# cbacary/MoDeGPT

Measured on AMD Instinct MI355X. Metric: transformer layers compressed/sec (covariance+decomp+rebuild), Llama-3-8B @30%, higher is better.
Workload: dtype f64 from int8 MFMA digit planes, exact route: nine plane pairs + fp64 remainder sums, nothing truncated (error <= 5e-15 per call: fp64 rounding)

## Files before the change

### modegpt_amd/csrc/cov_i8_exact.hip

```cpp
#include <algorithm>

#include "cov_i8.hpp"

namespace mdg {

struct __attribute__((aligned(16))) LoEntry {
  double v;
  unsigned off, aux;
};

namespace {

constexpr int LO_CHUNK_STEPS = 64;
constexpr int LO_CAP = 128;
constexpr double LO_ROUND = 8421504.0 / 16777216.0;
constexpr int EXACT_OVERFLOW = offsetof(SharedBlock, exact_overflow) / sizeof(int), EXACT_RAN = offsetof(SharedBlock, exact_ran) / sizeof(int),
              EXACT_MODE = offsetof(SharedBlock, exact_mode) / sizeof(int);
#ifndef MDG_LO_SPARSE_MEAN
#define MDG_LO_SPARSE_MEAN 32
#endif
#ifndef MDG_LO_SPARSE_MAX
#define MDG_LO_SPARSE_MAX 256
#endif
constexpr int LO_SPARSE_MAX = MDG_LO_SPARSE_MAX;
constexpr int LO_SUB = 4, LO_RCAP = 8 * LO_SPARSE_MAX;
constexpr int LO_TILE = 128, LO_PITCH = LO_TILE + 1;

struct LoProblem {
  const bf16_t* x;
  int64_t ld;
  const signed char* planes;
  const unsigned char* zmask;
  const int* emax;
  LoEntry* entries;
  int* counts;
  double* sigma;
  int64_t ld_sigma;
  bf16_t* xd;
  int n, block;
  LoEntry* rentries;
  int* rtotals;
  int tile0[3];
  int pairs;
};
struct LoArgs {
  LoProblem prob[MAX_PROBLEMS];
  int nprob, nk, nch, tiles[3];
  int64_t n_tokens;
  int always;
  const int* route_flag;
  int* state;
};
__device__ __forceinline__ int* lo_totals(const LoProblem& pr, int nch) { return pr.counts + (int64_t)pr.n * nch; }
constexpr int LO_AUTO_MIN_N = 4096;
__device__ __forceinline__ bool lo_offered(const LoArgs& a) {
  if (a.always) return true;
  if (a.prob[0].n >= LO_AUTO_MIN_N && !a.prob[0].block) return true;
  for (int p = 0; p < a.nprob; p++)
    if ((a.route_flag[p] & 3) == 1) return true;
  return false;
}

__global__ __launch_bounds__(64) void i8_extract_lo_kernel(LoArgs a) {
  const LoProblem& pr = a.prob[blockIdx.z];
  const int64_t groups = pr.n / 32;
  const int G = blockIdx.x, ch = blockIdx.y, lane = threadIdx.x;
  if (!lo_offered(a)) return;
  if (blockIdx.x == 0 && blockIdx.y == 0 && blockIdx.z == 0 && lane == 0) a.state[EXACT_RAN] = 1;
  if (G >= groups || (a.route_flag[blockIdx.z] & 2)) return;
  const int col = G * 32 + (lane & 31);
  LoEntry* out = pr.entries + ((int64_t)col * a.nch + ch) * LO_CAP;
  const double scale = ldexp(1.0, (pr.emax[col] & 255) - 172);
  int count = 0;
  const int kt1 = min(a.nk, (ch + 1) * LO_CHUNK_STEPS);
  for (int kt = ch * LO_CHUNK_STEPS; kt < kt1; kt++) {
    const unsigned m = pr.zmask[(int64_t)kt * groups + G];
    if ((m >> 3) == 0) continue;
    const i32x4 zero = (i32x4)0;
    const i32x4 d3 = *((const i32x4*)(pr.planes + ((3 * groups + G) * (int64_t)a.nk + kt) * 1024) + lane);
    const i32x4 d4 = (m >> 4) ? *((const i32x4*)(pr.planes + ((4 * groups + G) * (int64_t)a.nk + kt) * 1024) + lane) : zero;
    const i32x4 d5 = (m >> 5) ? *((const i32x4*)(pr.planes + ((5 * groups + G) * (int64_t)a.nk + kt) * 1024) + lane) : zero;
    const unsigned tok0 = (unsigned)kt * KS + (lane >> 5) * 16;
    int L[16], mine = 0;
#pragma unroll
    for (int q = 0; q < 16; q++) {
      const int sh = 8 * (q & 3);
      L[q] = (int)(signed char)((unsigned)d3[q >> 2] >> sh) * 65536 + (int)(signed char)((unsigned)d4[q >> 2] >> sh) * 256 +
             (int)(signed char)((unsigned)d5[q >> 2] >> sh);
      mine += L[q] != 0;
    }
    if (__ballot(mine != 0) == 0) continue;
    const int other = __shfl_xor(mine, 32);
    int at = count + ((lane >> 5) ? other : 0);
#pragma unroll
    for (int q = 0; q < 16; q++)
      if (L[q] != 0) {
        if (at < LO_CAP) out[at] = LoEntry{(double)L[q] * scale, (tok0 + q) * (unsigned)(pr.ld * 2), (tok0 + q) * (unsigned)(pr.n * 2)};
        at++;
      }
    count += mine + other;
  }
  if (lane < 32) {
    pr.counts[(int64_t)col * a.nch + ch] = min(count, LO_CAP);
    if (count > LO_CAP) a.state[EXACT_OVERFLOW] = 1;
  }
}

__global__ __launch_bounds__(64) void i8_compact_lo_kernel(LoArgs a) {
  if (!lo_offered(a) || a.state[EXACT_OVERFLOW] != 0) return;
  const LoProblem& pr = a.prob[blockIdx.y];
  const int col = blockIdx.x, lane = threadIdx.x;
  if (col >= pr.n || (a.route_flag[blockIdx.y] & 2)) return;
  const int* counts = pr.counts + (int64_t)col * a.nch;
  LoEntry* base = pr.entries + (int64_t)col * a.nch * LO_CAP;
  int total = 0;
  for (int ch = 0; ch < a.nch; ch++) {
    const int cnt = counts[ch];
    const LoEntry* src = base + (int64_t)ch * LO_CAP;
    if (total != ch * LO_CAP)
      for (int i = 0; i < cnt; i += 64) {
        LoEntry e = LoEntry{0., 0u, 0u};
        if (i + lane < cnt) e = src[i + lane];
        if (i + lane < cnt) base[total + i + lane] = e;
      }
    total += cnt;
  }
  if (lane == 0) lo_totals(pr, a.nch)[col] = total;
}

typedef unsigned u32x4 __attribute__((ext_vector_type(4)));
constexpr int LO_SPARSE_MEAN = MDG_LO_SPARSE_MEAN;
__global__ __launch_bounds__(1024) void i8_lo_mode_kernel(LoArgs a) {
  if (!lo_offered(a) || a.state[EXACT_OVERFLOW] != 0) return;
  __shared__ long long sums[16];
  __shared__ int maxs[16];
  long long sum = 0, cols = 0;
  int mx = 0;
  for (int p = 0; p < a.nprob; p++) {
    if (a.route_flag[p] & 2) continue;
    const LoProblem& pr = a.prob[p];
    cols += pr.n;
    for (int c = threadIdx.x; c < pr.n; c += 1024) {
      const int t = lo_totals(pr, a.nch)[c];
      sum += t;
      mx = max(mx, t);
    }
  }
  for (int o = 32; o; o >>= 1) {
    sum += __shfl_xor(sum, o);
    mx = max(mx, __shfl_xor(mx, o));
  }
  if ((threadIdx.x & 63) == 0) { sums[threadIdx.x >> 6] = sum; maxs[threadIdx.x >> 6] = mx; }
  __syncthreads();
  if (threadIdx.x == 0) {
    for (int w = 1; w < 16; w++) { sum += sums[w]; mx = max(mx, maxs[w]); }
    a.state[EXACT_MODE] = (mx <= LO_SPARSE_MAX && sum <= LO_SPARSE_MEAN * cols) ? 1 : 2;
  }
}

__global__ __launch_bounds__(64) void i8_residue_lo_kernel(LoArgs a) {
  if (a.state[EXACT_MODE] != 1) return;
  const LoProblem& pr = a.prob[blockIdx.y];
  const int id = blockIdx.x, lane = threadIdx.x;
  if (id >= pr.n / 32 * LO_SUB || (a.route_flag[blockIdx.y] & 2)) return;
  const int G = id / LO_SUB, sub = id % LO_SUB;
  LoEntry* out = pr.rentries + (int64_t)id * LO_RCAP;
  int at = 0;
  for (int k = 0; k < 8; k++) {
    const int col = G * 32 + 4 * k + sub;
    const int cnt = lo_totals(pr, a.nch)[col];
    for (int i = lane; i < cnt; i += 64) {
      LoEntry e = pr.entries[(int64_t)col * a.nch * LO_CAP + i];
      e.aux = 4 * k + sub;
      out[at + i] = e;
    }
    at += cnt;
  }
  if (lane == 0) pr.rtotals[id] = at;
}

template <class EL, bool RELU>
__global__ __launch_bounds__(256) void i8_copy_xd_kernel(LoArgs a) {
  if (a.state[EXACT_MODE] != 2) return;
  const LoProblem& pr = a.prob[blockIdx.y];
  if (a.route_flag[blockIdx.y] & 2) return;
  const int64_t per_row = pr.n / 8, total = a.n_tokens * per_row;
  for (int64_t i = (int64_t)blockIdx.x * 256 + threadIdx.x; i < total; i += (int64_t)gridDim.x * 256) {
    const int64_t t = i / per_row, c = (i - t * per_row) * 8;
    typedef unsigned u32x4u __attribute__((ext_vector_type(4), aligned(2)));
    const u32x4u v = *(const u32x4u*)(pr.x + t * pr.ld + c);
    *(u32x4*)(pr.xd + t * pr.n + c) = (u32x4){relu_pair<EL, RELU>(v[0]), relu_pair<EL, RELU>(v[1]), relu_pair<EL, RELU>(v[2]), relu_pair<EL, RELU>(v[3])};
  }
}
template <class EL, bool RELU>
__global__ __launch_bounds__(64) void i8_patch_xd_kernel(LoArgs a) {
  if (a.state[EXACT_MODE] != 2) return;
  const LoProblem& pr = a.prob[blockIdx.y];
  const int col = blockIdx.x, lane = threadIdx.x;
  if (col >= pr.n || (a.route_flag[blockIdx.y] & 2)) return;
  const int total = lo_totals(pr, a.nch)[col];
  const LoEntry* list = pr.entries + (int64_t)col * a.nch * LO_CAP;
  for (int i = lane; i < total; i += 64) {
    const LoEntry e = list[i];
    const double xd = EL::to_f64(*(const bf16_t*)((const char*)pr.x + e.off + 2 * col)) - e.v;
    *(bf16_t*)((char*)pr.xd + e.aux + 2 * col) = (bf16_t)EL::from_f64(xd);
  }
}

__device__ __forceinline__ void lds_add_f64(double* p, double v) {
  __hip_atomic_fetch_add(p, v, __ATOMIC_RELAXED, __HIP_MEMORY_SCOPE_WORKGROUP);
}
__device__ __forceinline__ int lo_perm(int i) { return (i >> 1) + 64 * (i & 1); }

constexpr int LO_UN = 32;
struct LoFirst {
  int cnt;
  LoEntry m;
};
__device__ __forceinline__ LoFirst lo_first(const LoProblem& pr, const int G, const int sub, const int lane) {
  const int list_id = G * LO_SUB + sub;
  LoFirst f;
  f.cnt = __builtin_amdgcn_readfirstlane(pr.rtotals[list_id]);
  f.m = LoEntry{0., 0u, 0u};
  if (f.cnt > 0) {
    f.m = pr.rentries[(int64_t)list_id * LO_RCAP + min(lane & (LO_UN - 1), f.cnt - 1)];
    if ((lane & (LO_UN - 1)) >= f.cnt) f.m.v = 0.;
  }
  return f;
}
template <class EL, bool RELU, bool COLS>
__device__ __forceinline__ void lo_events(const LoProblem& pr, const int nch, const int G, const int sub, const int partner0, const int g,
                                          const int lane, double* acc, const LoFirst& first) {
  const unsigned short* xs = (const unsigned short*)pr.x;
  unsigned lim_a = 0, lim_b = 0;
  double qa = 1., qb = 1., ia = 1., ib = 1.;
  if (COLS) {
    const int ea = pr.emax[partner0 + 2 * lane] & 255, eb = pr.emax[partner0 + 2 * lane + 1] & 255;
    qa = ldexp(1.0, ea - 148);
    qb = ldexp(1.0, eb - 148);
    ia = 1.0 / qa;
    ib = 1.0 / qb;
    lim_a = EL::deep_limit(ea);
    lim_b = EL::deep_limit(eb);
  }
  const int list_id = G * LO_SUB + sub;
  const int cnt = first.cnt;
  const LoEntry* list = pr.rentries + (int64_t)list_id * LO_RCAP;
  auto fetch = [&](int k, LoEntry& m) {
    m = list[min(k * LO_UN + (lane & (LO_UN - 1)), cnt - 1)];
    if (k * LO_UN + (lane & (LO_UN - 1)) >= cnt) m.v = 0.;
  };
  auto issue = [&](const LoEntry& m, unsigned (&xv)[LO_UN]) {
#pragma unroll
    for (int u = 0; u < LO_UN; u++) {
      const unsigned off = (unsigned)__builtin_amdgcn_readlane((int)m.off, u);
      const unsigned short* row = (const unsigned short*)((const char*)xs + off) + partner0 + 2 * lane;
      xv[u] = relu_pair<EL, RELU>(pr.pairs ? *(const unsigned*)row : ((unsigned)row[0] | ((unsigned)row[1] << 16)));
    }
  };
  auto multiply = [&](const LoEntry& m, const unsigned (&xv)[LO_UN]) {
#pragma unroll
    for (int u = 0; u < LO_UN; u++) {
      const double v = __hiloint2double(__builtin_amdgcn_readlane(__double2hiint(m.v), u), __builtin_amdgcn_readlane(__double2loint(m.v), u));
      const int col = __builtin_amdgcn_readlane((int)m.aux, u);
      double pa = EL::to_f64(xv[u] & 0xFFFFu), pb = EL::to_f64(xv[u] >> 16);
      if (COLS) {
        const bool deep = ((xv[u] & 0x7FFFu) - 1u < lim_a - 1u) || (((xv[u] >> 16) & 0x7FFFu) - 1u < lim_b - 1u);
        if (__ballot(deep)) {
          pa = floor(pa * ia + LO_ROUND) * qa;
          pb = floor(pb * ib + LO_ROUND) * qb;
        }
        lds_add_f64(acc + lane * LO_PITCH + lo_perm(g * 32 + col), v * pa);
        lds_add_f64(acc + (64 + lane) * LO_PITCH + lo_perm(g * 32 + col), v * pb);
      } else {
        lds_add_f64(acc + lo_perm(g * 32 + col) * LO_PITCH + lane, v * pa);
        lds_add_f64(acc + lo_perm(g * 32 + col) * LO_PITCH + 64 + lane, v * pb);
      }
    }
  };
  if (cnt == 0) return;
  const int nb = (cnt + LO_UN - 1) / LO_UN;
  LoEntry mA = first.m, mB;
  unsigned xA[LO_UN], xB[LO_UN];
  issue(mA, xA);
  for (int k = 0; k < nb; k += 2) {
    if (k + 1 < nb) {
      fetch(k + 1, mB);
      issue(mB, xB);
    }
    __builtin_amdgcn_sched_barrier(0);
    multiply(mA, xA);
    if (k + 1 >= nb) break;
    if (k + 2 < nb) {
      fetch(k + 2, mA);
      issue(mA, xA);
    }
    __builtin_amdgcn_sched_barrier(0);
    multiply(mB, xB);
  }
}

constexpr int LO_THREADS = 1024;
template <class EL, bool RELU>
__global__ __launch_bounds__(LO_THREADS) void i8_lo_product_kernel(LoArgs a) {
  extern __shared__ __attribute__((aligned(16))) double lo_acc[];
  if (a.state[EXACT_RAN] != 1 || a.state[EXACT_OVERFLOW] != 0 || a.state[EXACT_MODE] != 1) return;
  int p = 0;
  while (p + 1 < a.nprob && (int)blockIdx.x >= a.prob[p + 1].tile0[2]) p++;
  if (a.route_flag[p] & 2) return;
  const LoProblem& pr = a.prob[p];
  const int t = blockIdx.x - pr.tile0[2];
  int bi, bj;
  if (pr.block) {
    bi = bj = t;
  } else {
    bi = (int)((sqrtf(8.f * t + 1.f) - 1.f) * 0.5f);
    while ((bi + 1) * (bi + 2) / 2 <= t) bi++;
    while (bi * (bi + 1) / 2 > t) bi--;
    bj = t - bi * (bi + 1) / 2;
  }
  const int tid = threadIdx.x, lane = tid & 63;
  const int wave = __builtin_amdgcn_readfirstlane(tid >> 6);
  const int g = wave & 3, sub = wave >> 2;
  int any = 0;
  if (tid < 8 * LO_SUB) any = pr.rtotals[(tid < 4 * LO_SUB ? 4 * bi * LO_SUB : 4 * bj * LO_SUB - 4 * LO_SUB) + tid];
  if (!__syncthreads_or(any)) return;
  const LoFirst first_rows = lo_first(pr, 4 * bi + g, sub, lane), first_cols = lo_first(pr, 4 * bj + g, sub, lane);
  for (int i = tid; i < LO_TILE * LO_PITCH; i += LO_THREADS) lo_acc[i] = 0.;
  __syncthreads();
  lo_events<EL, RELU, false>(pr, a.nch, 4 * bi + g, sub, bj * LO_TILE, g, lane, lo_acc, first_rows);
  __syncthreads();
  lo_events<EL, RELU, true>(pr, a.nch, 4 * bj + g, sub, bi * LO_TILE, g, lane, lo_acc, first_cols);
  __syncthreads();
  constexpr int PER = LO_TILE * LO_TILE / LO_THREADS;
  const int c = tid % LO_TILE, col = bj * LO_TILE + c;
  const int e_col = col < pr.n ? pr.emax[col] : EMAX_COLUMN_OUT;
  double* s[PER];
  double old[PER], v[PER];
#pragma unroll
  for (int u = 0; u < PER; u++) {
    const int r = tid / LO_TILE + u * (LO_THREADS / LO_TILE), row = bi * LO_TILE + r;
    v[u] = lo_acc[lo_perm(r) * LO_PITCH + lo_perm(c)];
    const bool ours = col <= row && row < pr.n && v[u] != 0. && !((pr.emax[row] | e_col) & EMAX_COLUMN_OUT);
    s[u] = ours ? pr.sigma + (int64_t)row * pr.ld_sigma + col - (pr.block ? row / pr.block * pr.block : 0) : nullptr;
    old[u] = ours ? *s[u] : 0.;
  }
#pragma unroll
  for (int u = 0; u < PER; u++)
    if (s[u]) *s[u] = old[u] + v[u];
}

#ifndef MDG_LW_UN
#define MDG_LW_UN 8
#endif
#ifndef MDG_LW_OCC
#define MDG_LW_OCC 0
#endif
#if MDG_LW_OCC
#define LW_OCC_ATTR __attribute__((amdgpu_waves_per_eu(MDG_LW_OCC, MDG_LW_OCC)))
#else
#define LW_OCC_ATTR
#endif
constexpr int LW_COLS = 8, LW_BLOCK = 64 * LW_COLS, LW_UN = MDG_LW_UN, LW_GROUP = 16, LW_TP = LW_GROUP + 1;
template <class EL, bool RELU, bool TR>
__global__ __launch_bounds__(LO_THREADS) LW_OCC_ATTR void i8_lo_wide_kernel(LoArgs a) {
  if (a.state[EXACT_RAN] != 1 || a.state[EXACT_OVERFLOW] != 0 || a.state[EXACT_MODE] != 2) return;
  int p = 0;
  while (p + 1 < a.nprob && (int)blockIdx.x >= a.prob[p + 1].tile0[TR]) p++;
  if (a.route_flag[p] & 2) return;
  const LoProblem& pr = a.prob[p];
  const int n = pr.n, nG = n / LW_GROUP;
  constexpr int PER = LW_BLOCK / LW_GROUP;
  int t = blockIdx.x - pr.tile0[TR], G, P = 0;
  if (pr.block) {
    G = t;
  } else {
    for (;;) {
      const int cnt = TR ? min(nG, PER * (P + 1)) : nG - PER * P;
      if (t < cnt) break;
      t -= cnt;
      P++;
    }
    G = TR ? t : PER * P + t;
  }
  const int lane = threadIdx.x & 63;
  const int wave = __builtin_amdgcn_readfirstlane(threadIdx.x >> 6);
  const char* const xs = TR ? (const char*)pr.xd : (const char*)pr.x;
  typedef unsigned u32x4u __attribute__((ext_vector_type(4), aligned(2)));
  __shared__ double tr_tile[TR ? LW_BLOCK * LW_TP : 1];
  const int r = G * LW_GROUP + wave;
  const int total = __builtin_amdgcn_readfirstlane(lo_totals(pr, a.nch)[r]);
  const bool r_ours = total != 0 && !(pr.emax[r] & EMAX_COLUMN_OUT);
  const LoEntry* list = pr.entries + (int64_t)r * a.nch * LO_CAP;
  LoEntry m0 = LoEntry{0., 0u, 0u};
  if (r_ours) {
    m0 = list[min(lane, min(total, 64) - 1)];
    if (lane >= total) m0.v = 0.;
  }
  {
    const int p0 = pr.block ? G * LW_GROUP / pr.block * pr.block : P * LW_BLOCK;
    const int pend = pr.block ? p0 + pr.block : min(n, p0 + LW_BLOCK);
    const int c0 = p0 + LW_COLS * lane;
    unsigned mine = 0;
#pragma unroll
    for (int j = 0; j < LW_COLS; j++)
      if (c0 + j < pend && !(pr.emax[c0 + j] & EMAX_COLUMN_OUT) && (TR ? c0 + j >= r : c0 + j <= r)) mine |= 1u << j;
    const unsigned lane_off = (unsigned)(c0 + LW_COLS <= pend ? c0 : p0) * 2u;
    const bool walk = r_ours && __ballot(mine != 0) != 0;
    double acc[LW_COLS];
#pragma unroll
    for (int j = 0; j < LW_COLS; j++) acc[j] = 0.;
    if (walk) {
      for (int sb = 0; sb < total; sb += 64) {
        const int len = min(64, total - sb);
        LoEntry m = m0;
        if (sb) {
          m = list[sb + min(lane, len - 1)];
          if (lane >= len) m.v = 0.;
        }
        const unsigned moff = TR ? m.aux : m.off;
        u32x4 xa[LW_UN], xb[LW_UN];
        auto issue = [&](int b, u32x4 (&xv)[LW_UN]) {
#pragma unroll
          for (int u = 0; u < LW_UN; u++) {
            const unsigned o = (unsigned)__builtin_amdgcn_readlane((int)moff, b * LW_UN + u) + lane_off;
            const u32x4u q = *(const u32x4u*)(xs + o);
            xv[u] = (u32x4){q[0], q[1], q[2], q[3]};
          }
        };
        auto multiply = [&](int b, const u32x4 (&xv)[LW_UN]) {
#pragma unroll
          for (int u = 0; u < LW_UN; u++) {
            const double v = __hiloint2double(__builtin_amdgcn_readlane(__double2hiint(m.v), b * LW_UN + u),
                                              __builtin_amdgcn_readlane(__double2loint(m.v), b * LW_UN + u));
#pragma unroll
            for (int q = 0; q < 4; q++) {
              const unsigned w = TR ? xv[u][q] : relu_pair<EL, RELU>(xv[u][q]);
              acc[2 * q] = fma(v, EL::lo_f64(w), acc[2 * q]);
              acc[2 * q + 1] = fma(v, EL::hi_f64(w), acc[2 * q + 1]);
            }
          }
        };
        const int nb = (len + LW_UN - 1) / LW_UN;
        issue(0, xa);
        for (int b = 0; b < nb; b += 2) {
          __builtin_amdgcn_sched_barrier(0);
          if (b + 1 < nb) issue(b + 1, xb);
          __builtin_amdgcn_sched_barrier(0);
          multiply(b, xa);
          if (b + 1 >= nb) break;
          __builtin_amdgcn_sched_barrier(0);
          if (b + 2 < nb) issue(b + 2, xa);
          __builtin_amdgcn_sched_barrier(0);
          multiply(b + 1, xb);
        }
      }
    }
    if (!TR) {
      if (!walk) return;
      double* s[LW_COLS];
      double old[LW_COLS];
#pragma unroll
      for (int j = 0; j < LW_COLS; j++) {
        s[j] = (mine >> j & 1) ? pr.sigma + (int64_t)r * pr.ld_sigma + c0 + j - (pr.block ? r / pr.block * pr.block : 0) : nullptr;
        old[j] = s[j] ? *s[j] : 0.;
      }
#pragma unroll
      for (int j = 0; j < LW_COLS; j++)
        if (s[j]) *s[j] = old[j] + acc[j];
      return;
    }
#pragma unroll
    for (int j = 0; j < LW_COLS; j++) tr_tile[(LW_COLS * lane + j) * LW_TP + wave] = (walk && (mine >> j & 1)) ? acc[j] : 0.;
    __syncthreads();
    {
      const int i = p0 + (threadIdx.x >> 1), half = threadIdx.x & 1;
      if (i < pend && !(pr.emax[i] & EMAX_COLUMN_OUT)) {
        double v[8], old[8];
        double* s[8];
#pragma unroll
        for (int k = 0; k < 8; k++) {
          const int col = G * LW_GROUP + 8 * half + k;
          v[k] = tr_tile[(i - p0) * LW_TP + 8 * half + k];
          s[k] = (v[k] != 0. && col <= i) ? pr.sigma + (int64_t)i * pr.ld_sigma + col - (pr.block ? i / pr.block * pr.block : 0) : nullptr;
          old[k] = s[k] ? *s[k] : 0.;
        }
#pragma unroll
        for (int k = 0; k < 8; k++)
          if (s[k]) *s[k] = old[k] + v[k];
      }
    }
  }
}

template <bool TR>
void launch_lo_wide(const I8Call& c, const LoArgs& lo) {
  const dim3 grid((unsigned)lo.tiles[TR]), block(LO_THREADS);
  if (c.f16) {
    if (c.relu) hipLaunchKernelGGL((i8_lo_wide_kernel<F16Elem, true, TR>), grid, block, 0, c.st, lo);
    else hipLaunchKernelGGL((i8_lo_wide_kernel<F16Elem, false, TR>), grid, block, 0, c.st, lo);
  } else {
    if (c.relu) hipLaunchKernelGGL((i8_lo_wide_kernel<Bf16Elem, true, TR>), grid, block, 0, c.st, lo);
    else hipLaunchKernelGGL((i8_lo_wide_kernel<Bf16Elem, false, TR>), grid, block, 0, c.st, lo);
  }
}

int lo_chunks(int64_t T) { return (int)ceil_div(ceil_div(T, (int64_t)KS), (int64_t)LO_CHUNK_STEPS); }

LoArgs lo_args(const I8Call& c, bool always) {
  LoArgs lo;
  lo.nprob = c.count;
  lo.nk = c.nk;
  lo.nch = lo_chunks(c.n_tokens);
  lo.route_flag = c.shared->route_flag;
  lo.state = c.shared->reserved;
  lo.always = always ? 1 : 0;
  lo.n_tokens = c.n_tokens;
  int tiles[3] = {0, 0, 0};
  for (int i = 0; i < c.count; i++) {
    const I8Stat& s = c.stat[i];
    LoProblem& l = lo.prob[i];
    l.x = s.x; l.ld = s.ld;
    l.planes = s.planes; l.zmask = s.zmask; l.emax = s.emax;
    l.entries = s.lo_entries;
    l.xd = s.lo_xd;
    l.rentries = s.lo_rentries;
    l.rtotals = s.lo_rtotals;
    l.pairs = ((uintptr_t)s.x % 4 == 0) && (s.ld % 2 == 0);
    l.counts = s.lo_counts;
    l.sigma = s.sigma; l.ld_sigma = s.ld_sigma;
    l.n = s.n; l.block = s.block;
    const int nG = s.n / LW_GROUP, per = LW_BLOCK / LW_GROUP;
    for (int tr = 0; tr < 2; tr++) {
      l.tile0[tr] = tiles[tr];
      if (s.block) {
        tiles[tr] += nG;
      } else {
        for (int P = 0; P * per < nG; P++) tiles[tr] += tr ? std::min(nG, per * (P + 1)) : nG - per * P;
      }
    }
    l.tile0[2] = tiles[2];
    const int rbi = s.n / TI;
    tiles[2] += s.block ? rbi : rbi * (rbi + 1) / 2;
  }
  for (int i = c.count; i < MAX_PROBLEMS; i++) lo.prob[i] = lo.prob[0];
  for (int k = 0; k < 3; k++) lo.tiles[k] = tiles[k];
  return lo;
}

}

LoWsBytes lo_ws_bytes(int64_t n_tokens, int64_t n) {
  LoWsBytes b;
  b.entries = (size_t)n * lo_chunks(n_tokens) * LO_CAP * sizeof(LoEntry);
  b.counts = (size_t)n * (lo_chunks(n_tokens) + 1) * sizeof(int);
  b.xd = (size_t)n * (size_t)n_tokens * sizeof(bf16_t);
  b.rentries = (size_t)(n / 32) * LO_SUB * LO_RCAP * sizeof(LoEntry);
  b.rtotals = (size_t)(n / 32) * LO_SUB * sizeof(int);
  return b;
}

int enqueue_lo_lists(const I8Call& c, bool always) {
  const LoArgs lo = lo_args(c, always);
  int max_groups = 0;
  for (int i = 0; i < c.count; i++) max_groups = std::max(max_groups, c.stat[i].n / 32);
  const unsigned count = (unsigned)c.count;
  hipLaunchKernelGGL(i8_extract_lo_kernel, dim3((unsigned)max_groups, (unsigned)lo.nch, count), dim3(64), 0, c.st, lo);
  hipLaunchKernelGGL(i8_compact_lo_kernel, dim3((unsigned)(max_groups * 32), count), dim3(64), 0, c.st, lo);
  hipLaunchKernelGGL(i8_lo_mode_kernel, dim3(1), dim3(1024), 0, c.st, lo);
  hipLaunchKernelGGL(i8_residue_lo_kernel, dim3((unsigned)(max_groups * LO_SUB), count), dim3(64), 0, c.st, lo);
  MDG_I8_DISPATCH(c, i8_copy_xd_kernel, dim3(2048u, count), dim3(256), 0, c.st, lo);
  MDG_I8_DISPATCH(c, i8_patch_xd_kernel, dim3((unsigned)(max_groups * 32), count), dim3(64), 0, c.st, lo);
  MDG_LAUNCH_CHECK();
  return MDG_OK;
}

int enqueue_lo_products(const I8Call& c, bool always) {
  const LoArgs lo = lo_args(c, always);
  const size_t lds = (size_t)LO_TILE * LO_PITCH * sizeof(double);
  const void* tile_kernel = c.f16 ? (c.relu ? (const void*)i8_lo_product_kernel<F16Elem, true> : (const void*)i8_lo_product_kernel<F16Elem, false>)
                                  : (c.relu ? (const void*)i8_lo_product_kernel<Bf16Elem, true> : (const void*)i8_lo_product_kernel<Bf16Elem, false>);
  MDG_HIP(hipFuncSetAttribute(tile_kernel, hipFuncAttributeMaxDynamicSharedMemorySize, (int)lds));
  MDG_I8_DISPATCH(c, i8_lo_product_kernel, dim3((unsigned)lo.tiles[2]), dim3(LO_THREADS), lds, c.st, lo);
  launch_lo_wide<false>(c, lo);
  launch_lo_wide<true>(c, lo);
  MDG_LAUNCH_CHECK();
  return MDG_OK;
}

}
```

Measured before the change: 1.130.

## Prefetch sigma, emax and first entry batch before sync in low-product kernel

The low-precision remainder product kernel now loads the state flags, list lengths, emax values, the old sigma tile and the first batch of x rows up front, before the early-exit checks and barriers, so these global latencies overlap. The per-wave unroll drops from 32 to 16 entries, a first 64-entry head is reused from a single wave-wide load, and short lists skip the second half of each batch. Quantisation now uses ldexp instead of multiplying by precomputed scale factors. In exchange, blocks that will exit early still issue loads. The bounds checks on row and column against n are also removed, which relies on padding for out-of-range tiles.

```diff
diff --git a/modegpt_amd/csrc/cov_i8_exact.hip b/modegpt_amd/csrc/cov_i8_exact.hip
--- a/modegpt_amd/csrc/cov_i8_exact.hip
+++ b/modegpt_amd/csrc/cov_i8_exact.hip
@@ -212,91 +212,112 @@
 }
 __device__ __forceinline__ int lo_perm(int i) { return (i >> 1) + 64 * (i & 1); }
 
-constexpr int LO_UN = 32;
+constexpr int LO_UN = 16;
+#ifndef MDG_LO_SHORT
+#define MDG_LO_SHORT 8
+#endif
+constexpr int LO_SHORT = MDG_LO_SHORT;
+constexpr int LO_HEAD = 64;
 struct LoFirst {
   int cnt;
   LoEntry m;
 };
-__device__ __forceinline__ LoFirst lo_first(const LoProblem& pr, const int G, const int sub, const int lane) {
-  const int list_id = G * LO_SUB + sub;
+__device__ __forceinline__ LoFirst lo_first(const LoProblem& pr, const int list_id, const int cnt, const int lane) {
   LoFirst f;
-  f.cnt = __builtin_amdgcn_readfirstlane(pr.rtotals[list_id]);
-  f.m = LoEntry{0., 0u, 0u};
-  if (f.cnt > 0) {
-    f.m = pr.rentries[(int64_t)list_id * LO_RCAP + min(lane & (LO_UN - 1), f.cnt - 1)];
-    if ((lane & (LO_UN - 1)) >= f.cnt) f.m.v = 0.;
-  }
+  f.cnt = cnt;
+  f.m = pr.rentries[(int64_t)list_id * LO_RCAP + min(lane, max(cnt, 1) - 1)];
+  if (lane >= cnt) f.m.v = 0.;
   return f;
 }
+template <class EL, bool RELU, int U0, int U1>
+__device__ __forceinline__ void lo_issue_n(const LoProblem& pr, const unsigned m_off, const int e0, const int col0, unsigned (&xv)[LO_UN]) {
+  if (pr.pairs) {
+#pragma unroll
+    for (int u = U0; u < U1; u++) {
+      const unsigned off = (unsigned)__builtin_amdgcn_readlane((int)m_off, e0 + u);
+      xv[u] = relu_pair<EL, RELU>(*(const unsigned*)((const unsigned short*)((const char*)pr.x + off) + col0));
+    }
+  } else {
+#pragma unroll
+    for (int u = U0; u < U1; u++) {
+      const unsigned off = (unsigned)__builtin_amdgcn_readlane((int)m_off, e0 + u);
+      const unsigned short* row = (const unsigned short*)((const char*)pr.x + off) + col0;
+      xv[u] = relu_pair<EL, RELU>((unsigned)row[0] | ((unsigned)row[1] << 16));
+    }
+  }
+}
+constexpr int LO_FIRST_SLOTS = LO_SHORT ? LO_SHORT : LO_UN;
+template <class EL, bool RELU>
+__device__ __forceinline__ void lo_issue(const LoProblem& pr, const unsigned m_off, const int e0, const int left, const int col0,
+                                         unsigned (&xv)[LO_UN]) {
+  lo_issue_n<EL, RELU, 0, LO_FIRST_SLOTS>(pr, m_off, e0, col0, xv);
+  if (LO_SHORT && left > LO_SHORT) lo_issue_n<EL, RELU, LO_FIRST_SLOTS, LO_UN>(pr, m_off, e0, col0, xv);
+}
+template <class EL, bool COLS, int U0, int U1>
+__device__ __forceinline__ void lo_multiply_n(double* acc, const LoEntry& m, const int e0, const unsigned (&xv)[LO_UN], const int g, const int lane,
+                                              const int sa, const int sb, const unsigned lim_a, const unsigned lim_b) {
+#pragma unroll
+  for (int u = U0; u < U1; u++) {
+    const double v = __hiloint2double(__builtin_amdgcn_readlane(__double2hiint(m.v), e0 + u), __builtin_amdgcn_readlane(__double2loint(m.v), e0 + u));
+    const int col = __builtin_amdgcn_readlane((int)m.aux, e0 + u);
+    double pa = EL::to_f64(xv[u] & 0xFFFFu), pb = EL::to_f64(xv[u] >> 16);
+    if (COLS) {
+      const bool deep = ((xv[u] & 0x7FFFu) - 1u < lim_a - 1u) || (((xv[u] >> 16) & 0x7FFFu) - 1u < lim_b - 1u);
+      if (__ballot(deep)) {
+        pa = ldexp(floor(ldexp(pa, -sa) + LO_ROUND), sa);
+        pb = ldexp(floor(ldexp(pb, -sb) + LO_ROUND), sb);
+      }
+      lds_add_f64(acc + lane * LO_PITCH + lo_perm(g * 32 + col), v * pa);
+      lds_add_f64(acc + (64 + lane) * LO_PITCH + lo_perm(g * 32 + col), v * pb);
+    } else {
+      lds_add_f64(acc + lo_perm(g * 32 + col) * LO_PITCH + lane, v * pa);
+      lds_add_f64(acc + lo_perm(g * 32 + col) * LO_PITCH + 64 + lane, v * pb);
+    }
+  }
+}
 template <class EL, bool RELU, bool COLS>
-__device__ __forceinline__ void lo_events(const LoProblem& pr, const int nch, const int G, const int sub, const int partner0, const int g,
-                                          const int lane, double* acc, const LoFirst& first) {
-  const unsigned short* xs = (const unsigned short*)pr.x;
-  unsigned lim_a = 0, lim_b = 0;
-  double qa = 1., qb = 1., ia = 1., ib = 1.;
-  if (COLS) {
-    const int ea = pr.emax[partner0 + 2 * lane] & 255, eb = pr.emax[partner0 + 2 * lane + 1] & 255;
-    qa = ldexp(1.0, ea - 148);
-    qb = ldexp(1.0, eb - 148);
-    ia = 1.0 / qa;
-    ib = 1.0 / qb;
-    lim_a = EL::deep_limit(ea);
-    lim_b = EL::deep_limit(eb);
-  }
-  const int list_id = G * LO_SUB + sub;
+__device__ __forceinline__ void lo_events(const LoProblem& pr, const int list_id, const int partner0, const int g, const int lane, double* acc,
+                                          const LoFirst& first, const unsigned (&x0)[LO_UN], const int ea, const int eb) {
   const int cnt = first.cnt;
+  if (cnt == 0) return;
+  const int sa = (ea & 255) - 148, sb = (eb & 255) - 148;
+  const unsigned lim_a = COLS ? EL::deep_limit(ea & 255) : 0u, lim_b = COLS ? EL::deep_limit(eb & 255) : 0u;
+  const int col0 = partner0 + 2 * lane;
   const LoEntry* list = pr.rentries + (int64_t)list_id * LO_RCAP;
-  auto fetch = [&](int k, LoEntry& m) {
-    m = list[min(k * LO_UN + (lane & (LO_UN - 1)), cnt - 1)];
-    if (k * LO_UN + (lane & (LO_UN - 1)) >= cnt) m.v = 0.;
+  auto entries = [&](int k, LoEntry& m, int& e0) {
+    if (k < LO_HEAD / LO_UN) {
+      m = first.m;
+      e0 = k * LO_UN;
+    } else {
+      m = list[min(k * LO_UN + (lane & (LO_UN - 1)), cnt - 1)];
+      if (k * LO_UN + (lane & (LO_UN - 1)) >= cnt) m.v = 0.;
+      e0 = 0;
+    }
   };
-  auto issue = [&](const LoEntry& m, unsigned (&xv)[LO_UN]) {
-#pragma unroll
-    for (int u = 0; u < LO_UN; u++) {
-      const unsigned off = (unsigned)__builtin_amdgcn_readlane((int)m.off, u);
-      const unsigned short* row = (const unsigned short*)((const char*)xs + off) + partner0 + 2 * lane;
-      xv[u] = relu_pair<EL, RELU>(pr.pairs ? *(const unsigned*)row : ((unsigned)row[0] | ((unsigned)row[1] << 16)));
-    }
+  auto multiply = [&](const LoEntry& m, const int e0, const int left, const unsigned (&xv)[LO_UN]) {
+    lo_multiply_n<EL, COLS, 0, LO_FIRST_SLOTS>(acc, m, e0, xv, g, lane, sa, sb, lim_a, lim_b);
+    if (LO_SHORT && left > LO_SHORT) lo_multiply_n<EL, COLS, LO_FIRST_SLOTS, LO_UN>(acc, m, e0, xv, g, lane, sa, sb, lim_a, lim_b);
   };
-  auto multiply = [&](const LoEntry& m, const unsigned (&xv)[LO_UN]) {
-#pragma unroll
-    for (int u = 0; u < LO_UN; u++) {
-      const double v = __hiloint2double(__builtin_amdgcn_readlane(__double2hiint(m.v), u), __builtin_amdgcn_readlane(__double2loint(m.v), u));
-      const int col = __builtin_amdgcn_readlane((int)m.aux, u);
-      double pa = EL::to_f64(xv[u] & 0xFFFFu), pb = EL::to_f64(xv[u] >> 16);
-      if (COLS) {
-        const bool deep = ((xv[u] & 0x7FFFu) - 1u < lim_a - 1u) || (((xv[u] >> 16) & 0x7FFFu) - 1u < lim_b - 1u);
-        if (__ballot(deep)) {
-          pa = floor(pa * ia + LO_ROUND) * qa;
-          pb = floor(pb * ib + LO_ROUND) * qb;
-        }
-        lds_add_f64(acc + lane * LO_PITCH + lo_perm(g * 32 + col), v * pa);
-        lds_add_f64(acc + (64 + lane) * LO_PITCH + lo_perm(g * 32 + col), v * pb);
-      } else {
-        lds_add_f64(acc + lo_perm(g * 32 + col) * LO_PITCH + lane, v * pa);
-        lds_add_f64(acc + lo_perm(g * 32 + col) * LO_PITCH + 64 + lane, v * pb);
-      }
-    }
-  };
-  if (cnt == 0) return;
   const int nb = (cnt + LO_UN - 1) / LO_UN;
-  LoEntry mA = first.m, mB;
+  LoEntry mA = first.m, mB = first.m;
+  int eA = 0, eB = 0;
   unsigned xA[LO_UN], xB[LO_UN];
-  issue(mA, xA);
+#pragma unroll
+  for (int u = 0; u < LO_UN; u++) xA[u] = x0[u];
   for (int k = 0; k < nb; k += 2) {
     if (k + 1 < nb) {
-      fetch(k + 1, mB);
-      issue(mB, xB);
+      entries(k + 1, mB, eB);
+      lo_issue<EL, RELU>(pr, mB.off, eB, cnt - (k + 1) * LO_UN, col0, xB);
     }
     __builtin_amdgcn_sched_barrier(0);
-    multiply(mA, xA);
+    multiply(mA, eA, cnt - k * LO_UN, xA);
     if (k + 1 >= nb) break;
     if (k + 2 < nb) {
-      fetch(k + 2, mA);
-      issue(mA, xA);
+      entries(k + 2, mA, eA);
+      lo_issue<EL, RELU>(pr, mA.off, eA, cnt - (k + 2) * LO_UN, col0, xA);
     }
     __builtin_amdgcn_sched_barrier(0);
-    multiply(mB, xB);
+    multiply(mB, eB, cnt - (k + 1) * LO_UN, xB);
   }
 }
 
@@ -304,10 +325,8 @@
 template <class EL, bool RELU>
 __global__ __launch_bounds__(LO_THREADS) void i8_lo_product_kernel(LoArgs a) {
   extern __shared__ __attribute__((aligned(16))) double lo_acc[];
-  if (a.state[EXACT_RAN] != 1 || a.state[EXACT_OVERFLOW] != 0 || a.state[EXACT_MODE] != 1) return;
   int p = 0;
   while (p + 1 < a.nprob && (int)blockIdx.x >= a.prob[p + 1].tile0[2]) p++;
-  if (a.route_flag[p] & 2) return;
   const LoProblem& pr = a.prob[p];
   const int t = blockIdx.x - pr.tile0[2];
   int bi, bj;
@@ -322,32 +341,44 @@
   const int tid = threadIdx.x, lane = tid & 63;
   const int wave = __builtin_amdgcn_readfirstlane(tid >> 6);
   const int g = wave & 3, sub = wave >> 2;
-  int any = 0;
-  if (tid < 8 * LO_SUB) any = pr.rtotals[(tid < 4 * LO_SUB ? 4 * bi * LO_SUB : 4 * bj * LO_SUB - 4 * LO_SUB) + tid];
-  if (!__syncthreads_or(any)) return;
-  const LoFirst first_rows = lo_first(pr, 4 * bi + g, sub, lane), first_cols = lo_first(pr, 4 * bj + g, sub, lane);
+  constexpr int PER = LO_TILE * LO_TILE / LO_THREADS, ROWS = LO_THREADS / LO_TILE;
+  const int ran = a.state[EXACT_RAN], overflow = a.state[EXACT_OVERFLOW], mode = a.state[EXACT_MODE], flag = a.route_flag[p];
+  const int list_r = (4 * bi + g) * LO_SUB + sub, list_c = (4 * bj + g) * LO_SUB + sub;
+  const int len_r = pr.rtotals[list_r], len_c = pr.rtotals[list_c];
+  const int ea = pr.emax[bi * LO_TILE + 2 * lane], eb = pr.emax[bi * LO_TILE + 2 * lane + 1];
+  const int c = tid % LO_TILE, col = bj * LO_TILE + c, row0 = bi * LO_TILE + tid / LO_TILE;
+  const int e_col = pr.emax[col];
+  __builtin_amdgcn_sched_barrier(0);
+  if (ran != 1 || overflow != 0 || mode != 1 || (flag & 2)) return;
+  double* const sigma = pr.sigma;
+  const int64_t ld_sigma = pr.ld_sigma, at0 = (int64_t)row0 * ld_sigma + col - (pr.block ? bi * LO_TILE : 0);
+  double old[PER];
+#pragma unroll
+  for (int u = 0; u < PER; u++) {
+    const int64_t at = at0 + (int64_t)u * ROWS * ld_sigma;
+    old[u] = sigma[at & -(int64_t)(col <= row0 + u * ROWS)];
+  }
   for (int i = tid; i < LO_TILE * LO_PITCH; i += LO_THREADS) lo_acc[i] = 0.;
+  __builtin_amdgcn_sched_barrier(0);
+  const int cnt_r = __builtin_amdgcn_readfirstlane(len_r), cnt_c = __builtin_amdgcn_readfirstlane(len_c);
+  if (!__syncthreads_or(cnt_r | cnt_c)) return;
+  const LoFirst first_rows = lo_first(pr, list_r, cnt_r, lane), first_cols = lo_first(pr, list_c, cnt_c, lane);
+  unsigned x_rows[LO_UN], x_cols[LO_UN];
+  if (cnt_r) lo_issue<EL, RELU>(pr, first_rows.m.off, 0, cnt_r, bj * LO_TILE + 2 * lane, x_rows);
+  if (cnt_c) lo_issue<EL, RELU>(pr, first_cols.m.off, 0, cnt_c, bi * LO_TILE + 2 * lane, x_cols);
+  __builtin_amdgcn_sched_barrier(0);
+  lo_events<EL, RELU, false>(pr, list_r, bj * LO_TILE, g, lane, lo_acc, first_rows, x_rows, 0, 0);
   __syncthreads();
-  lo_events<EL, RELU, false>(pr, a.nch, 4 * bi + g, sub, bj * LO_TILE, g, lane, lo_acc, first_rows);
+  lo_events<EL, RELU, true>(pr, list_c, bi * LO_TILE, g, lane, lo_acc, first_cols, x_cols, ea, eb);
   __syncthreads();
-  lo_events<EL, RELU, true>(pr, a.nch, 4 * bj + g, sub, bi * LO_TILE, g, lane, lo_acc, first_cols);
-  __syncthreads();
-  constexpr int PER = LO_TILE * LO_TILE / LO_THREADS;
-  const int c = tid % LO_TILE, col = bj * LO_TILE + c;
-  const int e_col = col < pr.n ? pr.emax[col] : EMAX_COLUMN_OUT;
-  double* s[PER];
-  double old[PER], v[PER];
+  const int e_rows = (wave & 2) ? eb : ea;
 #pragma unroll
   for (int u = 0; u < PER; u++) {
-    const int r = tid / LO_TILE + u * (LO_THREADS / LO_TILE), row = bi * LO_TILE + r;
-    v[u] = lo_acc[lo_perm(r) * LO_PITCH + lo_perm(c)];
-    const bool ours = col <= row && row < pr.n && v[u] != 0. && !((pr.emax[row] | e_col) & EMAX_COLUMN_OUT);
-    s[u] = ours ? pr.sigma + (int64_t)row * pr.ld_sigma + col - (pr.block ? row / pr.block * pr.block : 0) : nullptr;
-    old[u] = ours ? *s[u] : 0.;
-  }
-#pragma unroll
-  for (int u = 0; u < PER; u++)
-    if (s[u]) *s[u] = old[u] + v[u];
+    const int r = tid / LO_TILE + u * ROWS, row = bi * LO_TILE + r;
+    const double v = lo_acc[lo_perm(r) * LO_PITCH + lo_perm(c)];
+    const int e_row = __builtin_amdgcn_readlane(e_rows, (wave >> 2) + u * (ROWS / 2));
+    if (col <= row && v != 0. && !((e_row | e_col) & EMAX_COLUMN_OUT)) sigma[at0 + (int64_t)u * ROWS * ld_sigma] = old[u] + v;
+  }
 }
 
 #ifndef MDG_LW_UN
```

After: 1.145, median of 6. +1.3%, better.
